# Stoffel-Labs/mpc-protocols

Measured on AMD Instinct MI355X. Metric: shares/sec (compute_shares) + recons/sec (batch_recon), 256-bit Fr, 1/2/4/8 GPU, higher is better.
Workload: dtype u32; 1 GPU; compute_shares n=16 t=5 batch=2^20 secrets per GPU (BASELINE configs[1]); field=bls12-381 Fr, parallelism=batch-sharded x1, no data-path collective, field_impl=u29

## Files before the change

mpc-protocols_amd/csrc/kernels_rng.hpp:

```cpp
#pragma once
#include <hip/hip_runtime.h>
#include <stdint.h>

#include "fr_consts.h"

namespace hbmpc {

struct SeedArg {
    uint32_t k[8];
};

__device__ __forceinline__ uint32_t rotl32(uint32_t v, int c) { return (v << c) | (v >> (32 - c)); }
#define HB_QR(a, b, c, d)                                   \
    a += b; d = rotl32(d ^ a, 16); c += d; b = rotl32(b ^ c, 12); \
    a += b; d = rotl32(d ^ a, 8);  c += d; b = rotl32(b ^ c, 7);

__device__ __forceinline__ void chacha20_block(const SeedArg& key, uint64_t counter, uint64_t nonce, uint32_t (&out)[16]) {
    const uint32_t in[16] = {0x61707865u, 0x3320646Eu, 0x79622D32u, 0x6B206574u, key.k[0], key.k[1], key.k[2], key.k[3],
                             key.k[4], key.k[5], key.k[6], key.k[7], (uint32_t)counter, (uint32_t)(counter >> 32),
                             (uint32_t)nonce, (uint32_t)(nonce >> 32)};
    uint32_t s0 = in[0], s1 = in[1], s2 = in[2], s3 = in[3], s4 = in[4], s5 = in[5], s6 = in[6], s7 = in[7], s8 = in[8], s9 = in[9],
             s10 = in[10], s11 = in[11], s12 = in[12], s13 = in[13], s14 = in[14], s15 = in[15];
#pragma unroll 2
    for (int r = 0; r < 10; ++r) {
        HB_QR(s0, s4, s8, s12) HB_QR(s1, s5, s9, s13) HB_QR(s2, s6, s10, s14) HB_QR(s3, s7, s11, s15)
        HB_QR(s0, s5, s10, s15) HB_QR(s1, s6, s11, s12) HB_QR(s2, s7, s8, s13) HB_QR(s3, s4, s9, s14)
    }
    const uint32_t s[16] = {s0, s1, s2, s3, s4, s5, s6, s7, s8, s9, s10, s11, s12, s13, s14, s15};
#pragma unroll
    for (int i = 0; i < 16; ++i) out[i] = s[i] + in[i];
}
#undef HB_QR

template <int EW>
__global__ __launch_bounds__(256) void k_fill_coeffs(SeedArg seed, const uint32_t* __restrict__ secrets, size_t B,
                                                     uint64_t first_index, int dp1, uint32_t* __restrict__ coeffs) {
    const size_t e = (size_t)blockIdx.x * blockDim.x + threadIdx.x;
    if (e >= B * (size_t)dp1) return;
    const size_t b = e / (size_t)dp1;
    const uint32_t k = (uint32_t)(e - b * (size_t)dp1);
    uint32_t* dst = coeffs + e * EW;
    if (k == 0 && secrets) {
#pragma unroll
        for (int w = 0; w < EW; ++w) dst[w] = secrets[b * EW + w];
        return;
    }
    for (uint32_t attempt = 0;; ++attempt) {
        uint32_t blk[16];
        chacha20_block(seed, ((uint64_t)k << 32) + attempt, first_index + b, blk);
#pragma unroll
        for (int c = 0; c < 16 / EW; ++c) {
            uint32_t v[EW];
#pragma unroll
            for (int w = 0; w < EW; ++w) v[w] = blk[c * EW + w];
            bool lt = false;
            if constexpr (EW == 8) {
                v[7] &= 0x7fffffffu;
#pragma unroll
                for (int w = 7; w >= 0; --w) {
                    if (v[w] != consts::S_MOD[w]) {
                        lt = v[w] < consts::S_MOD[w];
                        break;
                    }
                }
            } else {
                const uint64_t x = ((uint64_t)v[1] << 32) | v[0];
                lt = x < 0xFFFFFFFF00000001ull;
            }
            if (lt) {
#pragma unroll
                for (int w = 0; w < EW; ++w) dst[w] = v[w];
                return;
            }
        }
    }
}

}
```

mpc-protocols_amd/csrc/tu_rng.hip:

```cpp
#include "kernels_rng.hpp"
#include "launchers.hpp"
namespace hbmpc {
void launch_fill_coeffs(int ew, const uint32_t seed[8], const uint32_t* secrets, size_t B, uint64_t first_index, int dp1,
                        uint32_t* coeffs, hipStream_t s) {
    SeedArg k;
    for (int i = 0; i < 8; ++i) k.k[i] = seed[i];
    const size_t total = B * (size_t)dp1;
    const unsigned grid = (unsigned)((total + 255) / 256);
    if (ew == 8) hipLaunchKernelGGL((k_fill_coeffs<8>), dim3(grid), dim3(256), 0, s, k, secrets, B, first_index, dp1, coeffs);
    else hipLaunchKernelGGL((k_fill_coeffs<2>), dim3(grid), dim3(256), 0, s, k, secrets, B, first_index, dp1, coeffs);
}
}
```

Measured before the change: 144.1 billion shares/s.

## Restructure coefficient fill into per-block runs with LDS retry queues

Reworks the ChaCha-based coefficient fill kernel. Each workgroup now owns a tile of secrets-by-coefficients, and every thread handles several elements in a grid-stride loop. Rejected draws are pushed onto double-buffered LDS queues and retried level by level, so a wave no longer diverges on per-lane retry loops. The per-chunk modulus comparison becomes a branch-free inline-asm subtract-borrow chain, and one draw now tests both 256-bit candidates and stores with 16-byte pieces. The costs are block-wide syncs per retry level, extra LDS use, and reciprocal-based index math.

```diff
diff --git a/mpc-protocols_amd/csrc/kernels_rng.hpp b/mpc-protocols_amd/csrc/kernels_rng.hpp
--- a/mpc-protocols_amd/csrc/kernels_rng.hpp
+++ b/mpc-protocols_amd/csrc/kernels_rng.hpp
@@ -3,6 +3,7 @@
 #include <stdint.h>
 
 #include "fr_consts.h"
+#include "rng_fill_plan.hpp"
 
 namespace hbmpc {
 
@@ -32,47 +33,102 @@
 }
 #undef HB_QR
 
+struct __attribute__((packed, aligned(8))) FillPiece16 {
+    uint32_t w[4];
+};
+
+__device__ __forceinline__ uint32_t fr_below_modulus(const uint32_t* v) {
+    uint32_t t, lt;
+    asm("v_sub_co_u32_e32 %0, vcc, %10, %2\n\t"
+        "v_subb_co_u32_e32 %0, vcc, %11, %3, vcc\n\t"
+        "v_subb_co_u32_e32 %0, vcc, %12, %4, vcc\n\t"
+        "v_subb_co_u32_e32 %0, vcc, %13, %5, vcc\n\t"
+        "v_subb_co_u32_e32 %0, vcc, %14, %6, vcc\n\t"
+        "v_subb_co_u32_e32 %0, vcc, %15, %7, vcc\n\t"
+        "v_subb_co_u32_e32 %0, vcc, %16, %8, vcc\n\t"
+        "v_subb_co_u32_e32 %0, vcc, %17, %9, vcc\n\t"
+        "v_cndmask_b32_e64 %1, 0, 1, vcc"
+        : "=&v"(t), "=v"(lt)
+        : "v"(consts::S_MOD[0]), "v"(consts::S_MOD[1]), "v"(consts::S_MOD[2]), "v"(consts::S_MOD[3]), "v"(consts::S_MOD[4]),
+          "v"(consts::S_MOD[5]), "v"(consts::S_MOD[6]), "v"(consts::S_MOD[7]), "v"(v[0]), "v"(v[1]), "v"(v[2]), "v"(v[3]), "v"(v[4]),
+          "v"(v[5]), "v"(v[6]), "v"(v[7])
+        : "vcc");
+    return lt;
+}
+
+template <int EW>
+__device__ __forceinline__ bool fill_draw(const SeedArg& seed, uint64_t nonce, uint32_t k, uint32_t attempt, uint32_t* __restrict__ dst) {
+    uint32_t blk[16];
+    chacha20_block(seed, ((uint64_t)k << 32) + attempt, nonce, blk);
+    if constexpr (EW == 8) {
+        blk[7] &= 0x7fffffffu;
+        blk[15] &= 0x7fffffffu;
+        const uint32_t br0 = fr_below_modulus(&blk[0]), br1 = fr_below_modulus(&blk[8]);
+        if (!(br0 | br1)) return false;
+        FillPiece16 lo, hi;
+#pragma unroll
+        for (int w = 0; w < 4; ++w) {
+            lo.w[w] = br0 ? blk[w] : blk[8 + w];
+            hi.w[w] = br0 ? blk[4 + w] : blk[12 + w];
+        }
+        ((FillPiece16*)dst)[0] = lo;
+        ((FillPiece16*)dst)[1] = hi;
+        return true;
+    } else {
+        uint64_t pick = 0;
+        bool any = false;
+#pragma unroll
+        for (int c = 7; c >= 0; --c) {
+            const uint64_t x = ((uint64_t)blk[2 * c + 1] << 32) | blk[2 * c];
+            const bool lt = x < 0xFFFFFFFF00000001ull;
+            pick = lt ? x : pick;
+            any |= lt;
+        }
+        if (!any) return false;
+        *(uint64_t*)dst = pick;
+        return true;
+    }
+}
+
 template <int EW>
 __global__ __launch_bounds__(256) void k_fill_coeffs(SeedArg seed, const uint32_t* __restrict__ secrets, size_t B,
-                                                     uint64_t first_index, int dp1, uint32_t* __restrict__ coeffs) {
-    const size_t e = (size_t)blockIdx.x * blockDim.x + threadIdx.x;
-    if (e >= B * (size_t)dp1) return;
-    const size_t b = e / (size_t)dp1;
-    const uint32_t k = (uint32_t)(e - b * (size_t)dp1);
-    uint32_t* dst = coeffs + e * EW;
-    if (k == 0 && secrets) {
-#pragma unroll
-        for (int w = 0; w < EW; ++w) dst[w] = secrets[b * EW + w];
-        return;
+                                                     uint64_t first_index, FillPlan p, uint32_t* __restrict__ coeffs) {
+    extern __shared__ __attribute__((aligned(16))) unsigned char fill_lds[];
+    uint32_t* cnt = (uint32_t*)fill_lds;
+    uint16_t* const queue[2] = {(uint16_t*)(fill_lds + kFillQueueOffset), (uint16_t*)(fill_lds + kFillQueueOffset + fill_queue_bytes(p))};
+    const uint32_t tid = threadIdx.x;
+    const size_t b0 = (size_t)blockIdx.x * p.tb;
+    const uint32_t nb = (uint32_t)(B - b0 < (size_t)p.tb ? B - b0 : (size_t)p.tb);
+    const uint32_t k0 = blockIdx.y * p.kc;
+    const uint32_t nk = p.dd - k0 < p.kc ? p.dd - k0 : p.kc;
+    const uint32_t run = nb * nk;
+    if (tid < kFillCounters) cnt[tid] = 0;
+    uint32_t* const run_rows = coeffs + b0 * p.dp1 * EW;
+    const uint64_t nonce0 = first_index + b0;
+    auto element = [&](uint32_t j, uint32_t attempt) {
+        const uint32_t row = fill_elem_row(p, j), k = p.kfirst + fill_elem_kk(p, j, k0, row);
+        if (!fill_draw<EW>(seed, nonce0 + row, k, attempt, run_rows + (size_t)((row * p.dp1 + k) * EW)))
+            queue[fill_queue(attempt + 1)][atomicAdd(&cnt[fill_counter(attempt + 1)], 1u)] = (uint16_t)j;
+    };
+    __syncthreads();
+    for (uint32_t j = tid; j < run; j += kFillLanes) element(j, 0);
+    if (secrets && blockIdx.y == 0) {
+        if constexpr (EW == 8) {
+            for (uint32_t i = tid; i < 2 * nb; i += kFillLanes) {
+                const size_t b = b0 + (i >> 1);
+                ((FillPiece16*)(coeffs + b * p.dp1 * EW))[i & 1] = ((const FillPiece16*)(secrets + b * EW))[i & 1];
+            }
+        } else {
+            for (uint32_t i = tid; i < nb; i += kFillLanes) *(uint64_t*)(coeffs + (b0 + i) * p.dp1 * EW) = *(const uint64_t*)(secrets + (b0 + i) * EW);
+        }
     }
-    for (uint32_t attempt = 0;; ++attempt) {
-        uint32_t blk[16];
-        chacha20_block(seed, ((uint64_t)k << 32) + attempt, first_index + b, blk);
-#pragma unroll
-        for (int c = 0; c < 16 / EW; ++c) {
-            uint32_t v[EW];
-#pragma unroll
-            for (int w = 0; w < EW; ++w) v[w] = blk[c * EW + w];
-            bool lt = false;
-            if constexpr (EW == 8) {
-                v[7] &= 0x7fffffffu;
-#pragma unroll
-                for (int w = 7; w >= 0; --w) {
-                    if (v[w] != consts::S_MOD[w]) {
-                        lt = v[w] < consts::S_MOD[w];
-                        break;
-                    }
-                }
-            } else {
-                const uint64_t x = ((uint64_t)v[1] << 32) | v[0];
-                lt = x < 0xFFFFFFFF00000001ull;
-            }
-            if (lt) {
-#pragma unroll
-                for (int w = 0; w < EW; ++w) dst[w] = v[w];
-                return;
-            }
-        }
+    for (uint32_t level = 1;; ++level) {
+        __syncthreads();
+        const uint32_t n = cnt[fill_counter(level)];
+        if (n == 0) break;
+        if (tid == 0) cnt[fill_counter(level + 2)] = 0;
+        const uint16_t* q = queue[fill_queue(level)];
+        for (uint32_t i = tid; i < n; i += kFillLanes) element(q[i], level);
     }
 }
 
diff --git a/mpc-protocols_amd/csrc/rng_fill_plan.hpp b/mpc-protocols_amd/csrc/rng_fill_plan.hpp
--- /dev/null
+++ b/mpc-protocols_amd/csrc/rng_fill_plan.hpp
@@ -0,0 +1,67 @@
+#pragma once
+#include <stddef.h>
+#include <stdint.h>
+
+namespace hbmpc {
+
+constexpr uint32_t kFillLanes = 256;
+constexpr uint32_t kFillRoundsMax = 10;
+constexpr uint32_t kFillRunMax = kFillLanes * kFillRoundsMax;
+constexpr uint32_t kFillWgsTarget = 2048;
+constexpr uint32_t kFillCounters = 3;
+constexpr uint32_t kFillQueueOffset = 16;
+
+struct FillPlan {
+    uint32_t dd;
+    uint32_t kfirst;
+    uint32_t dp1;
+    uint32_t tb;
+    uint32_t kc;
+    uint32_t chunks;
+    uint32_t recip;
+    uint32_t qcap;
+};
+
+inline FillPlan fill_plan_rounds(uint32_t rounds, size_t d, bool has_secrets) {
+    FillPlan p;
+    p.dd = (uint32_t)d + (has_secrets ? 0u : 1u);
+    p.kfirst = has_secrets ? 1u : 0u;
+    p.dp1 = (uint32_t)d + 1u;
+    const uint32_t run = rounds * kFillLanes;
+    if (p.dd <= run) {
+        p.tb = run / (p.dd ? p.dd : 1u);
+        p.kc = p.dd;
+        p.chunks = 1;
+    } else {
+        p.tb = 1;
+        p.kc = run;
+        p.chunks = (p.dd + run - 1) / run;
+    }
+    p.recip = p.dd ? (uint32_t)((((uint64_t)1 << 31) + p.dd - 1) / p.dd) : 0u;
+    p.qcap = p.tb * p.kc;
+    return p;
+}
+
+inline uint32_t fill_rounds(size_t B, size_t d, bool has_secrets) {
+    const size_t total = B * (d + (has_secrets ? 0u : 1u)), share = (size_t)kFillLanes * kFillWgsTarget;
+    const size_t rounds = (total + share - 1) / share;
+    return rounds < 1 ? 1u : rounds > kFillRoundsMax ? kFillRoundsMax : (uint32_t)rounds;
+}
+inline FillPlan fill_plan(size_t B, size_t d, bool has_secrets) { return fill_plan_rounds(fill_rounds(B, d, has_secrets), d, has_secrets); }
+
+inline size_t fill_grid_x(const FillPlan& p, size_t B) { return (B + p.tb - 1) / p.tb; }
+
+constexpr uint32_t fill_elem_row(const FillPlan& p, uint32_t j) {
+    return p.chunks > 1 ? 0u : (uint32_t)(((uint64_t)(2u * j) * p.recip) >> 32);
+}
+constexpr uint32_t fill_elem_kk(const FillPlan& p, uint32_t j, uint32_t k0, uint32_t row) { return p.chunks > 1 ? k0 + j : j - row * p.dd; }
+
+constexpr uint32_t fill_queue(uint32_t level) { return level & 1u; }
+constexpr uint32_t fill_counter(uint32_t level) { return level % kFillCounters; }
+constexpr size_t fill_queue_bytes(const FillPlan& p) { return ((size_t)p.qcap * 2 + 15) & ~(size_t)15; }
+constexpr size_t fill_lds_bytes(const FillPlan& p) { return kFillQueueOffset + 2 * fill_queue_bytes(p); }
+
+static_assert(kFillRunMax <= 65536, "a queue entry is a 16-bit element number");
+static_assert(kFillCounters * 4 <= kFillQueueOffset, "the counters lie before the queues");
+
+}
diff --git a/mpc-protocols_amd/csrc/tu_rng.hip b/mpc-protocols_amd/csrc/tu_rng.hip
--- a/mpc-protocols_amd/csrc/tu_rng.hip
+++ b/mpc-protocols_amd/csrc/tu_rng.hip
@@ -5,9 +5,10 @@
                         uint32_t* coeffs, hipStream_t s) {
     SeedArg k;
     for (int i = 0; i < 8; ++i) k.k[i] = seed[i];
-    const size_t total = B * (size_t)dp1;
-    const unsigned grid = (unsigned)((total + 255) / 256);
-    if (ew == 8) hipLaunchKernelGGL((k_fill_coeffs<8>), dim3(grid), dim3(256), 0, s, k, secrets, B, first_index, dp1, coeffs);
-    else hipLaunchKernelGGL((k_fill_coeffs<2>), dim3(grid), dim3(256), 0, s, k, secrets, B, first_index, dp1, coeffs);
+    const FillPlan p = fill_plan(B, (size_t)dp1 - 1, secrets != nullptr);
+    const dim3 grid((unsigned)fill_grid_x(p, B), p.chunks);
+    const size_t lds = fill_lds_bytes(p);
+    if (ew == 8) hipLaunchKernelGGL((k_fill_coeffs<8>), grid, dim3(kFillLanes), lds, s, k, secrets, B, first_index, p, coeffs);
+    else hipLaunchKernelGGL((k_fill_coeffs<2>), grid, dim3(kFillLanes), lds, s, k, secrets, B, first_index, p, coeffs);
 }
 }
```

Result: no change. 143.4 billion shares/s (-0.4%).
